# HaoxiangYou/Q_Learning_with_HJB

Measured on AMD Instinct MI355X. Metric: env-steps/sec (batched HJB rollouts), cartpole batch=2^20, higher is better.
Workload: dtype f32; 1 GPU; cartpole balancing + vhjb controller (BASELINE configs[1]); batch_per_gpu=1048576, global_batch=1048576, state_dim=4, control_dim=1, integrator=euler, mlp=4-128-128-64 relu, no bias, parallelism=env-shard x1, no data-path collective

## Files before the change

q_learning_with_hjb_amd/csrc/hjbx_train_coop.hip:

```cpp
#include <hip/hip_runtime.h>
#include <type_traits>

#include "hjbx_internal.hpp"
#include "hjbx_systems.hpp"
#include "hjbx_host.hpp"
#include "hjbx_mlp_core.hpp"
#include "hjbx_adam.hpp"

using namespace hjbx;

static constexpr int kExLd = 33;
static constexpr int kExFloats = 128 * kExLd;
static constexpr int kCoopBlocks = 48;
static constexpr int kCoopSet = 24;
static constexpr int kCoopMaxGrid = 512;

template <int N> struct CoopLds {
    static constexpr int NP = (N + 3) & ~3;
    float W1[N * kLD1];
    float W2[kH1 * kLD2];
    float W3[kH2 * kLD3];
    float E[3][kExFloats];
    __attribute__((aligned(16))) float zs[32 * NP];
    __attribute__((aligned(16))) float gzbs[32 * NP];
    float rs[32];
    float vp[2][32];
    float zeros[32];
    double sums[4][32];
};

template <int AOFF, int BOFF, int ST> __device__ __forceinline__ void coop_issue(float& a, float& b, uint32_t abase, uint32_t bbase) {
    a = lds_read_b32<AOFF * ST>(abase);
    b = lds_read_b32<BOFF * ST>(bbase);
}
struct NoFiller { template <typename I> __device__ __forceinline__ void operator()(I) const {} };
template <int AOFF, int BOFF, int NSTEPS, int DEPTH, int ST, typename Filler>
__device__ __forceinline__ void coop_chain_step(f32x16& acc, float (&ra)[DEPTH + 1], float (&rb)[DEPTH + 1], uint32_t abase, uint32_t bbase, const Filler& filler) {
    if constexpr (ST < NSTEPS) {
        if constexpr (ST + DEPTH < NSTEPS) coop_issue<AOFF, BOFF, ST + DEPTH>(ra[(ST + DEPTH) % (DEPTH + 1)], rb[(ST + DEPTH) % (DEPTH + 1)], abase, bbase);
        __builtin_amdgcn_sched_barrier(0);
        constexpr int ahead = (NSTEPS - 1 - ST < DEPTH ? NSTEPS - 1 - ST : DEPTH) * 2;
        lds_wait<ahead>();
        acc = MFMA(ra[ST % (DEPTH + 1)], rb[ST % (DEPTH + 1)], acc);
        __builtin_amdgcn_sched_barrier(0);
        filler(std::integral_constant<int, ST>{});
        coop_chain_step<AOFF, BOFF, NSTEPS, DEPTH, ST + 1>(acc, ra, rb, abase, bbase, filler);
    }
}
template <int AOFF, int BOFF, int NSTEPS, typename Filler = NoFiller>
__device__ __forceinline__ void coop_chain(f32x16& acc, uint32_t abase, uint32_t bbase, const Filler& filler = Filler()) {
    constexpr int DEPTH = 3;
    static_assert(AOFF * (NSTEPS - 1) < 65536 && BOFF * (NSTEPS - 1) < 65536, "ds_read_b32 offset field is 16 bits");
    float ra[DEPTH + 1], rb[DEPTH + 1];
    coop_issue<AOFF, BOFF, 0>(ra[0], rb[0], abase, bbase);
    if constexpr (NSTEPS > 1) coop_issue<AOFF, BOFF, 1>(ra[1], rb[1], abase, bbase);
    if constexpr (NSTEPS > 2) coop_issue<AOFF, BOFF, 2>(ra[2], rb[2], abase, bbase);
    coop_chain_step<AOFF, BOFF, NSTEPS, DEPTH, 0>(acc, ra, rb, abase, bbase, filler);
}

struct OffW1Fc { static constexpr int at(int st, int) { return 2 * st * kLD1 * 4; } };
struct OffW1Gc { static constexpr int at(int st, int) { return perm(st) * 4; } };

using LP = __attribute__((address_space(3))) float*;
using LPc = const __attribute__((address_space(3))) float*;
__device__ __forceinline__ uint32_t lds_addr(LPc q) { return (uint32_t)(uintptr_t)q; }

__device__ __forceinline__ void zero16(f32x16& a) {
#pragma unroll
    for (int r = 0; r < 16; ++r) a[r] = 0.f;
}

__device__ __forceinline__ void ex_write(LP blk , const f32x16& v) {
#pragma unroll
    for (int r = 0; r < 16; ++r) blk[perm(r) * kExLd] = v[r];
}
__device__ __forceinline__ void ex_add(f32x16& v, LPc blk) {
#pragma unroll
    for (int r = 0; r < 16; ++r) v[r] += blk[perm(r) * kExLd];
}

template <int NB, bool HJB, bool TERM, typename Filler = NoFiller>
__device__ __forceinline__ void coop_outer(f32x16 (&acch)[NB], LPc Ah, LPc Bh, f32x16 (&acct)[NB], LPc At, LPc Bt, LPc rs, int exA, int exBj, int h,
                                           const Filler& filler = Filler()) {
    LPc ah_p = Ah + exA, bh_p = Bh + exBj, at_p = At + exA, bt_p = Bt + exBj, r_p = rs + h;
    struct Ops { float ah, at, rr, bh[NB], bt[NB]; };
    auto load = [&](int s2) __attribute__((always_inline)) {
        Ops o;
        o.ah = o.at = o.rr = 0.f;
        if constexpr (HJB) o.ah = ah_p[2 * s2];
        if constexpr (TERM) { o.at = at_p[2 * s2]; o.rr = r_p[2 * s2]; }
#pragma unroll
        for (int j = 0; j < NB; ++j) {
            o.bh[j] = o.bt[j] = 0.f;
            if constexpr (HJB) o.bh[j] = bh_p[32 * j * kExLd + 2 * s2];
            if constexpr (TERM) o.bt[j] = bt_p[32 * j * kExLd + 2 * s2];
        }
        return o;
    };
    Ops cur = load(0);
#pragma unroll
    for (int s = 0; s < 16; ++s) {
        Ops nxt = cur;
        if (s + 1 < 16) nxt = load(s + 1);
        __builtin_amdgcn_sched_barrier(0);
#pragma unroll
        for (int j = 0; j < NB; ++j) {
            if constexpr (HJB) acch[j] = MFMA(cur.ah, cur.bh[j], acch[j]);
            if constexpr (TERM) acct[j] = MFMA(cur.at, cur.rr * cur.bt[j], acct[j]);
        }
        filler(s);
        __builtin_amdgcn_sched_barrier(0);
        cur = nxt;
    }
}

#ifdef HJBX_COOP_NO_OUTER
#define COOP_OUTER(...)
#else
#define COOP_OUTER(...) __VA_ARGS__
#endif
#ifdef HJBX_COOP_NO_CHAINS
#define COOP_CHAIN(...)
#else
#define COOP_CHAIN(...) __VA_ARGS__
#endif
#ifdef HJBX_COOP_NO_BARRIER
#define COOP_SYNC() __builtin_amdgcn_sched_barrier(0)
#elif defined(HJBX_COOP_STAMPS)
#define COOP_STAMP() do { if (stamp_on) stamp_buf[stamp_idx++] = wall_clock64(); } while (0)
#define COOP_SYNC() do { __syncthreads(); COOP_STAMP(); } while (0)
#else
#define COOP_SYNC() __syncthreads()
#endif
#ifndef COOP_STAMP
#define COOP_STAMP() do { } while (0)
#endif

template <int MODE, int ACT, int PS, typename S>
__global__ __launch_bounds__(256, 1) void k_train_coop(S sys_k, MlpP<S::N> p_k, TaskP<float, S::N, S::M> tk_k, Limits<float, S::M> lim_k,
                                                       const float* __restrict__ W1g, const float* __restrict__ W2g, const float* __restrict__ W3g,
                                                       const float* __restrict__ x, const float* __restrict__ cost, const float* __restrict__ done,
                                                       float eps_term, float* __restrict__ partial, float* __restrict__ partial_w1,
                                                       double* __restrict__ sums_rec, int64_t B, int64_t ntiles) {
    constexpr int N = S::N, M = S::M;
    constexpr int NP = CoopLds<N>::NP;
    static_assert(N % 2 == 0 && N <= HJBX_MAX_N, "state dimension");
    __shared__ __attribute__((aligned(256))) CoopLds<N> L;
    __shared__ __attribute__((aligned(16))) unsigned char sys_raw[sizeof(S)];
    S& sys_s = *reinterpret_cast<S*>(sys_raw);
    __shared__ MlpP<N> p_s;
    __shared__ TaskP<float, N, M> tk_s;
    __shared__ Limits<float, M> lim_s;
    const int tid = threadIdx.x;
#ifdef HJBX_COOP_STAMPS
    const bool stamp_on = PS == 4 && blockIdx.x == 1 && tid == 0;
    unsigned long long* stamp_buf = reinterpret_cast<unsigned long long*>(partial_w1 + (int64_t)blockIdx.x * 2 * (2 * S::N * 128));
    int stamp_idx = 0;
    COOP_STAMP();
#endif
    if (tid == 0) { sys_s = sys_k; p_s = p_k; tk_s = tk_k; lim_s = lim_k; }
#ifndef HJBX_COOP_NO_FILL
    {
        static_assert(kH1 % 4 == 0 && kH2 % 4 == 0 && kH3 % 4 == 0, "");
        const float4* W1v = reinterpret_cast<const float4*>(W1g);
        const float4* W2v = reinterpret_cast<const float4*>(W2g);
        const float4* W3v = reinterpret_cast<const float4*>(W3g);
        auto put4 = [](float* dst, const float4& v) { dst[0] = v.x; dst[1] = v.y; dst[2] = v.z; dst[3] = v.w; };
        constexpr int Q1 = (N * kH1 / 4 + 255) / 256, Q2 = kH1 * kH2 / 4 / 256, Q3 = kH2 * kH3 / 4 / 256;
        static_assert(kH1 * kH2 / 4 % 256 == 0 && kH2 * kH3 / 4 % 256 == 0, "");
        float4 v1[Q1], v2[Q2], v3[Q3];
#pragma unroll
        for (int q = 0; q < Q2; ++q) v2[q] = W2v[tid + 256 * q];
#pragma unroll
        for (int q = 0; q < Q3; ++q) v3[q] = W3v[tid + 256 * q];
#pragma unroll
        for (int q = 0; q < Q1; ++q) v1[q] = tid + 256 * q < N * kH1 / 4 ? W1v[tid + 256 * q] : float4{0.f, 0.f, 0.f, 0.f};
#pragma unroll
        for (int q = 0; q < Q1; ++q) {
            const int idx = tid + 256 * q;
            if (idx < N * kH1 / 4) put4(&L.W1[(idx / (kH1 / 4)) * kLD1 + 4 * (idx % (kH1 / 4))], v1[q]);
        }
#pragma unroll
        for (int q = 0; q < Q2; ++q) { const int idx = tid + 256 * q; put4(&L.W2[(idx / (kH2 / 4)) * kLD2 + 4 * (idx % (kH2 / 4))], v2[q]); }
#pragma unroll
        for (int q = 0; q < Q3; ++q) { const int idx = tid + 256 * q; put4(&L.W3[(idx / (kH3 / 4)) * kLD3 + 4 * (idx % (kH3 / 4))], v3[q]); }
    }
#endif
    if (tid < 32) L.zeros[tid] = 0.f;
    if (tid < 128) L.sums[tid >> 5][tid & 31] = 0.0;
    for (int idx = tid; idx < kExFloats; idx += 256) L.E[2][idx] = 0.f;
    for (int idx = tid; idx < 32 * NP; idx += 256) { L.zs[idx] = 0.f; L.gzbs[idx] = 0.f; }
    __syncthreads();
    COOP_STAMP();
    const S& sys = sys_s;
    const MlpP<N>& p = p_s;
    const TaskP<float, N, M>& tk = tk_s;
    const Limits<float, M>& lim = lim_s;
    const int lane = tid & 63, w = __builtin_amdgcn_readfirstlane(tid >> 6);
    const int i = lane & 31, h = lane >> 5;
    const int ob = w & 1, kh = w >> 1;
    static_assert(PS == 1 || PS == 4, "");
    constexpr int psplit = PS;
    constexpr int NB2 = PS == 4 ? 1 : 4, NB3 = PS == 4 ? 1 : 2;
    const int part = PS == 4 ? (int)(blockIdx.x & 3u) : 0;
    const int col2 = PS == 4 ? 32 * part * kExLd : 0;
    const int col3 = PS == 4 ? 32 * (part & 1) * kExLd : 0;
    const bool do3 = PS == 1 || part < 2;
    const bool own1 = part == 0;
    const float m1 = own1 ? 1.0f : 0.0f;
    auto lds = [](const void* q) { return (uint32_t)(uintptr_t)q; };
    auto lds3 = [](LPc q) { return lds_addr(q); };
    const uint32_t aW1f = lds(&L.W1[h * kLD1 + 32 * w + i]);
    const uint32_t aW1g = i < N ? lds(&L.W1[i * kLD1 + 32 * w + 4 * h]) : lds(&L.zeros[0]);
    const uint32_t aW2f = lds(&L.W2[h * kLD2 + 32 * w + i]);
    const uint32_t aW2b = lds(&L.W2[(32 * w + i) * kLD2 + h]);
    const uint32_t aW3f = lds(&L.W3[(64 * kh + h) * kLD3 + 32 * ob + i]);
    const uint32_t aW3b = lds(&L.W3[(32 * w + i) * kLD3 + h]);
    const LP E0g = (LP)&L.E[0][0], E1g = (LP)&L.E[1][0], E2g = (LP)&L.E[2][0];
    const LP rsg = (LP)&L.rs[0], zsg = (LP)&L.zs[0], gzbsg = (LP)&L.gzbs[0];
    const int exB = h * kExLd + i;
    const int exW = (32 * w + 4 * h) * kExLd + i;
    const int exWy = (32 * ob + 4 * h) * kExLd + i;
    const int exA = (32 * w + i) * kExLd + h;
    const int exO = i * kExLd + h;
    constexpr int AO1 = 2 * kLD2 * 4, AO3 = 2 * kLD3 * 4, BOX = 2 * kExLd * 4;

    f32x16 acc2h[NB2], acc2t[NB2], acc3h[NB3], acc3t[NB3];
#pragma unroll
    for (int j = 0; j < NB2; ++j) { zero16(acc2h[j]); zero16(acc2t[j]); }
#pragma unroll
    for (int j = 0; j < NB3; ++j) { zero16(acc3h[j]); zero16(acc3t[j]); }
    f32x2 w1h[N / 2], w1t[N / 2];
#pragma unroll
    for (int k = 0; k < N / 2; ++k) w1h[k] = w1t[k] = f32x2{0.f, 0.f};
    const int fW1 = tid & 127, sW1 = 16 * (tid >> 7);

    auto fetch = [&](int64_t tile, float (&xv)[N], float& dnv, float& cstv) __attribute__((always_inline)) {
        const int64_t env = tile * 32 + i;
        const bool ok = tile < ntiles && env < B;
        if (ok) load_row<N>(x, env, xv);
        else {
#pragma unroll
            for (int k = 0; k < N; ++k) xv[k] = p.xf[k];
        }
        dnv = ok ? done[env] : 0.f;
        cstv = ok ? cost[env] : 1.f;
    };
    float xs_n[N], dn_n, cst_n;
    const int64_t tile_stride = gridDim.x / (unsigned)psplit;
    fetch(blockIdx.x / (unsigned)psplit, xs_n, dn_n, cst_n);
    for (int64_t tile = blockIdx.x / (unsigned)psplit; tile < ntiles; tile += tile_stride) {
        asm volatile("" ::: "memory");
        LP E0 = E0g, E1 = E1g, E2 = E2g, rsp = rsg, zsp = zsg, gzbsp = gzbsg;
        asm volatile("" : "+v"(E0), "+v"(E1), "+v"(E2), "+v"(rsp), "+v"(zsp), "+v"(gzbsp));
        const bool valid = tile * 32 + i < B;
        float xs[N];
#pragma unroll
        for (int k = 0; k < N; ++k) xs[k] = xs_n[k];
        const float dn = dn_n, cst = cst_n;
        float e[N], z[N], ee = 0.f;
#pragma unroll
        for (int k = 0; k < N; ++k) e[k] = xs[k] - p.xf[k];
        sys.wrap(e);
#pragma unroll
        for (int k = 0; k < N; ++k) {
            ee += e[k] * e[k];
            z[k] = (e[k] - p.mean[k]) * p.istd[k];
        }
        float ring1[3][1];
        f32x16 t[1][1];

        zero_acc(t);
        mfma_chain<OffW1Fc, N / 2, 1, 2, 1>(t, ring1, aW1f, [&](int st, int) { return h ? z[2 * st + 1] : z[2 * st]; });
        constexpr bool SIN = ACT == HJBX_ACT_SIN;
        f32x16 h1r, s1r;
#pragma unroll
        for (int r = 0; r < 16; ++r) {
            if constexpr (SIN) {
                float sn, cs;
                sincos1(t[0][0][r], sn, cs);
                asm volatile("" : "+v"(sn), "+v"(cs));
                h1r[r] = sn;
                s1r[r] = cs;
            } else {
                h1r[r] = act1<ACT>(t[0][0][r]);
            }
        }
        auto dmul1 = [&](int r, float v) __attribute__((always_inline)) { if constexpr (SIN) return v * s1r[r]; else return dact1<ACT>(h1r[r], v); };
        ex_write(E0 + exW, h1r);
        COOP_SYNC();
        f32x16 acc;
        zero16(acc);
        {
            using f32x4 = __attribute__((ext_vector_type(4))) float;
            using LP4 = const __attribute__((address_space(3))) f32x4*;
            LPc a1p = E2 + fW1 * kExLd + sW1;
            const LP4 zz4 = (LP4)(zsp + sW1 * NP);
            auto w1_part2 = [&](auto st_c) __attribute__((always_inline)) {
                constexpr int st = decltype(st_c)::value;
#if !defined(HJBX_COOP_NO_W1) && !defined(HJBX_COOP_NO_FILL2)
                if constexpr (st % 4 == 0) {
                    constexpr int s2 = st / 4;
                    const float a = a1p[s2] * m1;
                    const f32x2 a2v{a, a};
#pragma unroll
                    for (int k4 = 0; k4 < NP / 4; ++k4) {
                        const f32x4 zz = zz4[s2 * (NP / 4) + k4];
#pragma unroll
                        for (int c = 0; c < 2; ++c)
                            if (4 * k4 + 2 * c < N) w1h[2 * k4 + c] = __builtin_elementwise_fma(f32x2{zz[2 * c], zz[2 * c + 1]}, a2v, w1h[2 * k4 + c]);
                    }
#pragma unroll
                    for (int k = 0; k < N / 2; ++k) asm volatile("" : "+v"(w1h[k]));
                }
#endif
            };
#ifdef HJBX_COOP_NO_CHAINS
            (void)w1_part2;
#endif
            COOP_CHAIN(coop_chain<AO1, BOX, 64>(acc, aW2f, lds3(E0 + exB), w1_part2);)
        }
        f32x16 h2r, s2r;
#pragma unroll
        for (int r = 0; r < 16; ++r) {
            if constexpr (SIN) {
                float sn, cs;
                sincos1(acc[r], sn, cs);
                asm volatile("" : "+v"(sn), "+v"(cs));
                h2r[r] = sn;
                s2r[r] = cs;
            } else {
                h2r[r] = act1<ACT>(acc[r]);
            }
        }
        auto dmul2 = [&](int r, float v) __attribute__((always_inline)) { if constexpr (SIN) return v * s2r[r]; else return dact1<ACT>(h2r[r], v); };
        ex_write(E1 + exW, h2r);
        COOP_SYNC();
        zero16(acc);
        COOP_CHAIN(coop_chain<AO3, BOX, 32>(acc, aW3f, lds3(E1 + 64 * kh * kExLd + exB));)
        if (kh == 1) ex_write(E2 + exWy, acc);
        COOP_SYNC();
        f32x16 dyr;
        zero16(dyr);
        if (kh == 0) {
            ex_add(acc, E2 + exWy);
            float vpart = 0.f;
#pragma unroll
            for (int r = 0; r < 16; ++r) {
                vpart += acc[r] * acc[r];
                dyr[r] = acc[r] + acc[r];
            }
            vpart += __shfl_xor(vpart, 32, 64);
            if (h == 0) L.vp[ob][i] = vpart;
            ex_write(E0 + exWy, dyr);
        }
        COOP_SYNC();
        const float V = (L.vp[0][i] + L.vp[1][i]) + p.eps_s * ee;
        float lt, rterm;
        termination_residual_env<float>(eps_term, V, cst, dn, lt, rterm);
        if (!valid) lt = rterm = 0.f;
        if (w == 0 && h == 0) {
            L.rs[i] = rterm;
            if (valid && own1) { L.sums[1][i] += (double)lt; L.sums[2][i] += 1.0 - (double)dn; L.sums[3][i] += (double)dn; }
        }
        zero16(acc);
        COOP_CHAIN(coop_chain<2 * 4, BOX, 32>(acc, aW3b, lds3(E0 + exB));)
        f32x16 d2r;
        f32x16 c2r;
#pragma unroll
        for (int r = 0; r < 16; ++r) {
            d2r[r] = dmul2(r, acc[r]);
            if constexpr (SIN) c2r[r] = -h2r[r] * acc[r];
        }
        ex_write(E1 + exW, d2r);
        COOP_SYNC();
        zero16(acc);
        COOP_CHAIN(coop_chain<2 * 4, BOX, 64>(acc, aW2b, lds3(E1 + exB));)
        f32x16 d1r;
        f32x16 c1r;
#pragma unroll
        for (int r = 0; r < 16; ++r) {
            d1r[r] = dmul1(r, acc[r]);
            if constexpr (SIN) c1r[r] = -h1r[r] * acc[r];
        }
        ex_write(E2 + exW, d1r);
        zero_acc(t);
        mfma_chain<OffW1Gc, 16, 1, 2, 1>(t, ring1, aW1g, [&](int st, int) { return d1r[st]; });
        {
            LP gp = E0 + w * (N * 32) + i;
#pragma unroll
            for (int r = 0; r < 16; ++r) {
                const int k0 = perm(r);
                if (k0 + 4 * h < N && (k0 < N)) gp[(k0 + 4 * h) * 32] = t[0][0][r];
            }
        }
        COOP_SYNC();
        float g[N];
#pragma unroll
        for (int k = 0; k < N; ++k) {
            LPc gp = E0 + k * 32 + i;
            g[k] = ((gp[0] + gp[N * 32]) + (gp[2 * N * 32] + gp[3 * N * 32])) * p.istd[k] + 2.f * p.eps_s * e[k];
        }
        float li, q[N];
#ifdef HJBX_COOP_NO_RESID
        li = g[0];
#pragma unroll
        for (int k = 0; k < N; ++k) q[k] = g[k];
#else
        hjb_residual_env<MODE>(sys, tk, lim, xs, g, dn, true, li, q);
#endif
        if (!valid) {
            li = 0.f;
#pragma unroll
            for (int k = 0; k < N; ++k) q[k] = 0.f;
        }
        float gzb[N];
#pragma unroll
        for (int k = 0; k < N; ++k) gzb[k] = q[k] * p.istd[k];
        if (w == 0 && h == 0) {
            if (valid && own1) L.sums[0][i] += (double)li;
#pragma unroll
            for (int k = 0; k < N; ++k) { L.zs[i * NP + k] = z[k]; L.gzbs[i * NP + k] = gzb[k]; }
        }
        zero_acc(t);
        mfma_chain<OffW1Fc, N / 2, 1, 2, 1>(t, ring1, aW1f, [&](int st, int) { return h ? gzb[2 * st + 1] : gzb[2 * st]; });
        f32x16 dh1b;
#pragma unroll
        for (int r = 0; r < 16; ++r) {
            if constexpr (ACT == HJBX_ACT_TANH) c1r[r] = -2.f * h1r[r] * d1r[r] * t[0][0][r];
            if constexpr (SIN) c1r[r] *= t[0][0][r];
            dh1b[r] = dmul1(r, t[0][0][r]);
        }
        COOP_SYNC();
        ex_write(E0 + exW, dh1b);
        COOP_SYNC();
        using f32x4 = __attribute__((ext_vector_type(4))) float;
        using LP4 = const __attribute__((address_space(3))) f32x4*;
        LPc d1p = E2 + fW1 * kExLd + sW1, rp1 = rsp + sW1;
        const LP4 gz4 = (LP4)(gzbsp + sW1 * NP), zz4 = (LP4)(zsp + sW1 * NP);
        auto w1_part1 = [&](int s2) __attribute__((always_inline)) {
#if !defined(HJBX_COOP_NO_W1) && !defined(HJBX_COOP_NO_FILL1)
            const float d = d1p[s2] * m1;
            const float rd = rp1[s2] * d;
            const f32x2 d2v{d, d}, rd2v{rd, rd};
#pragma unroll
            for (int k4 = 0; k4 < NP / 4; ++k4) {
                const f32x4 gz = gz4[s2 * (NP / 4) + k4];
                const f32x4 zz = zz4[s2 * (NP / 4) + k4];
#pragma unroll
                for (int c = 0; c < 2; ++c)
                    if (4 * k4 + 2 * c < N) {
                        w1h[2 * k4 + c] = __builtin_elementwise_fma(f32x2{gz[2 * c], gz[2 * c + 1]}, d2v, w1h[2 * k4 + c]);
                        w1t[2 * k4 + c] = __builtin_elementwise_fma(f32x2{zz[2 * c], zz[2 * c + 1]}, rd2v, w1t[2 * k4 + c]);
                    }
            }
#pragma unroll
            for (int k = 0; k < N / 2; ++k) asm volatile("" : "+v"(w1h[k]), "+v"(w1t[k]));
#endif
        };
#ifdef HJBX_COOP_NO_OUTER
#pragma unroll
        for (int s2 = 0; s2 < 16; ++s2) w1_part1(s2);
#endif
        COOP_OUTER(coop_outer<NB2, true, false>(acc2h, E0, E1 + col2, acc2t, E0, E1 + col2, rsp, exA, exO, h, w1_part1);)
        zero16(acc);
        COOP_CHAIN(coop_chain<AO1, BOX, 64>(acc, aW2f, lds3(E0 + exB));)
        f32x16 dh2b;
#pragma unroll
        for (int r = 0; r < 16; ++r) {
            if constexpr (ACT == HJBX_ACT_TANH) c2r[r] = -2.f * h2r[r] * d2r[r] * acc[r];
            if constexpr (SIN) c2r[r] *= acc[r];
            dh2b[r] = dmul2(r, acc[r]);
        }
        COOP_SYNC();
        ex_write(E1 + exW, dh2b);
        if (kh == 0) ex_write(E2 + exWy, dyr);
        COOP_SYNC();
        COOP_OUTER(coop_outer<NB3, true, false>(acc3h, E1, E2 + col3, acc3t, E1, E2 + col3, rsp, exA, exO, h);)
        fetch(tile + tile_stride, xs_n, dn_n, cst_n);
        zero16(acc);
        COOP_CHAIN(coop_chain<AO3, BOX, 32>(acc, aW3f, lds3(E1 + 64 * kh * kExLd + exB));)
        if (kh == 1) ex_write(E0 + exWy, acc);
        COOP_SYNC();
        if (kh == 0) {
            ex_add(acc, E0 + exWy);
#pragma unroll
            for (int r = 0; r < 16; ++r) acc[r] += acc[r];
            ex_write(E0 + exWy, acc);
        }
        ex_write(E1 + exW, h2r);
        COOP_SYNC();
        COOP_OUTER(coop_outer<NB3, true, true>(acc3h, E1, E0 + col3, acc3t, E1, E2 + col3, rsp, exA, exO, h);)
        zero16(acc);
        COOP_CHAIN(coop_chain<2 * 4, BOX, 32>(acc, aW3b, lds3(E0 + exB));)
        f32x16 a2b;
#pragma unroll
        for (int r = 0; r < 16; ++r) {
            a2b[r] = dmul2(r, acc[r]);
            if constexpr (ACT != HJBX_ACT_RELU) a2b[r] += c2r[r];
        }
        COOP_SYNC();
        ex_write(E2 + exW, a2b);
        ex_write(E1 + exW, h1r);
        ex_write(E0 + exW, d2r);
        COOP_SYNC();
        COOP_OUTER(coop_outer<NB2, true, true>(acc2h, E1, E2 + col2, acc2t, E1, E0 + col2, rsp, exA, exO, h);)
        zero16(acc);
        COOP_CHAIN(coop_chain<2 * 4, BOX, 64>(acc, aW2b, lds3(E2 + exB));)
        f32x16 a1b;
#pragma unroll
        for (int r = 0; r < 16; ++r) {
            a1b[r] = dmul1(r, acc[r]);
            if constexpr (ACT != HJBX_ACT_RELU) a1b[r] += c1r[r];
        }
        COOP_SYNC();
        ex_write(E2 + exW, a1b);
    }
    COOP_SYNC();
    {
        using f32x4 = __attribute__((ext_vector_type(4))) float;
        using LP4 = const __attribute__((address_space(3))) f32x4*;
        LPc a1p = E2g + fW1 * kExLd + sW1;
        const LP4 zz4 = (LP4)(zsg + sW1 * NP);
#ifndef HJBX_COOP_NO_W1
#pragma unroll 4
        for (int s2 = 0; s2 < 16; ++s2) {
            const float a = a1p[s2] * m1;
            const f32x2 a2v{a, a};
#pragma unroll
            for (int k4 = 0; k4 < NP / 4; ++k4) {
                const f32x4 zz = zz4[s2 * (NP / 4) + k4];
#pragma unroll
                for (int c = 0; c < 2; ++c)
                    if (4 * k4 + 2 * c < N) w1h[2 * k4 + c] = __builtin_elementwise_fma(f32x2{zz[2 * c], zz[2 * c + 1]}, a2v, w1h[2 * k4 + c]);
            }
        }
#endif
    }
    COOP_STAMP();
    float* out = partial + (int64_t)blockIdx.x * kCoopBlocks * 1024;
    auto put = [&](int blk, const f32x16& a) {
#pragma unroll
        for (int r = 0; r < 16; ++r) out[blk * 1024 + r * 64 + lane] = a[r];
    };
    if constexpr (PS == 4) {
        put(w * 4 + part, acc2h[0]);
        put(kCoopSet + w * 4 + part, acc2t[0]);
        if (do3) {
            put(16 + w * 2 + (part & 1), acc3h[0]);
            put(kCoopSet + 16 + w * 2 + (part & 1), acc3t[0]);
        }
    } else {
#pragma unroll
        for (int j = 0; j < NB2; ++j) { put(w * 4 + j, acc2h[j]); put(kCoopSet + w * 4 + j, acc2t[j]); }
#pragma unroll
        for (int j = 0; j < NB3; ++j) { put(16 + w * 2 + j, acc3h[j]); put(kCoopSet + 16 + w * 2 + j, acc3t[j]); }
    }
    if (own1) {
        float* o1 = partial_w1 + ((int64_t)blockIdx.x * 2 + (tid >> 7)) * (2 * N * 128);
#pragma unroll
        for (int k = 0; k < N; ++k) { o1[k * 128 + fW1] = w1h[k >> 1][k & 1]; o1[(N + k) * 128 + fW1] = w1t[k >> 1][k & 1]; }
    }
    if (w == 0 && own1) {
        double acc_h = h == 0 ? L.sums[0][i] : 0.0, acc_t = h == 0 ? L.sums[1][i] : 0.0;
        double acc_ni = h == 0 ? L.sums[2][i] : 0.0, acc_nd = h == 0 ? L.sums[3][i] : 0.0;
#pragma unroll
        for (int off = 32; off > 0; off >>= 1) {
            acc_h += __shfl_down(acc_h, off, 64); acc_t += __shfl_down(acc_t, off, 64);
            acc_ni += __shfl_down(acc_ni, off, 64); acc_nd += __shfl_down(acc_nd, off, 64);
        }
        if (lane == 0) {
            double* rec = sums_rec + 4 * (int64_t)blockIdx.x;
            rec[0] = acc_h; rec[1] = acc_t; rec[2] = acc_ni; rec[3] = acc_nd;
        }
    }
    COOP_STAMP();
#ifdef HJBX_COOP_STAMPS
    if (stamp_on) stamp_buf[63] = (unsigned long long)stamp_idx;
#endif
}

__device__ __forceinline__ float coop_sum8(const float* __restrict__ base, int64_t stride, int count) {
    float s8[8] = {0.f, 0.f, 0.f, 0.f, 0.f, 0.f, 0.f, 0.f};
    int gI = 0;
    for (; gI + 8 <= count; gI += 8) {
#pragma unroll
        for (int k = 0; k < 8; ++k) s8[k] += base[(int64_t)(gI + k) * stride];
    }
    for (int k = 0; gI < count; ++gI, ++k) s8[k] += base[(int64_t)gI * stride];
    return ((s8[0] + s8[1]) + (s8[2] + s8[3])) + ((s8[4] + s8[5]) + (s8[6] + s8[7]));
}
__device__ __forceinline__ void coop_sum8x2(const float* __restrict__ a, const float* __restrict__ b, int64_t stride, int count, float& sa, float& sb) {
    float p[8] = {0.f, 0.f, 0.f, 0.f, 0.f, 0.f, 0.f, 0.f}, q[8] = {0.f, 0.f, 0.f, 0.f, 0.f, 0.f, 0.f, 0.f};
    int gI = 0;
    for (; gI + 8 <= count; gI += 8) {
        float va[8], vb[8];
#pragma unroll
        for (int k = 0; k < 8; ++k) { va[k] = a[(int64_t)(gI + k) * stride]; vb[k] = b[(int64_t)(gI + k) * stride]; }
#pragma unroll
        for (int k = 0; k < 8; ++k) { p[k] += va[k]; q[k] += vb[k]; }
    }
    for (int k = 0; gI < count; ++gI, ++k) { p[k] += a[(int64_t)gI * stride]; q[k] += b[(int64_t)gI * stride]; }
    sa = ((p[0] + p[1]) + (p[2] + p[3])) + ((p[4] + p[5]) + (p[6] + p[7]));
    sb = ((q[0] + q[1]) + (q[2] + q[3])) + ((q[4] + q[5]) + (q[6] + q[7]));
}

template <int N> __device__ __forceinline__ float coop_sum_w1(const float* __restrict__ base , int nparts, int psplit) {
    if (psplit != 4) return coop_sum8(base, 2 * N * 128, 2 * nparts);
    float s0, s1;
    coop_sum8x2(base, base + 2 * N * 128, (int64_t)8 * (2 * N * 128), nparts / 4, s0, s1);
    return s0 + s1;
}

struct CoopOwners { int first, step, count; };
__device__ __forceinline__ CoopOwners coop_owners(int b , int nparts, int psplit) {
    if (psplit != 4) return CoopOwners{0, 1, nparts};
    const int jb = b < 0 ? 0 : (b < 16 ? (b & 3) : ((b - 16) & 1));
    return CoopOwners{jb, 4, nparts / 4};
}

template <int N>
__global__ __launch_bounds__(256) void k_train_coop_reduce(const float* __restrict__ partial, const float* __restrict__ partial_w1, int nparts, int psplit,
                                                          const double* __restrict__ sums_rec, float* __restrict__ flat) {
    constexpr int P = N * kH1 + kH1 * kH2 + kH2 * kH3;
    const int t = blockIdx.x * 256 + threadIdx.x;
    if (t < kCoopBlocks * 1024) {
        const CoopOwners ow = coop_owners((t >> 10) % kCoopSet, nparts, psplit);
        const float s = coop_sum8(partial + (int64_t)ow.first * kCoopBlocks * 1024 + t, (int64_t)ow.step * kCoopBlocks * 1024, ow.count);
        const int blk = t >> 10, reg = (t >> 6) & 15, lane = t & 63;
        const int row = (reg & 3) + 8 * (reg >> 2) + 4 * (lane >> 5), col = lane & 31;
        const int set = blk / kCoopSet, b = blk % kCoopSet;
        float* o = flat + set * P;
        if (b < 16) o[N * kH1 + (32 * (b >> 2) + row) * kH2 + 32 * (b & 3) + col] = s;
        else o[N * kH1 + kH1 * kH2 + (32 * ((b - 16) >> 1) + row) * kH3 + 32 * ((b - 16) & 1) + col] = s;
    } else if (t < kCoopBlocks * 1024 + 2 * N * 128) {
        const int u = t - kCoopBlocks * 1024;
        const int set = u / (N * 128), kf = u % (N * 128);
        flat[set * P + kf] = coop_sum_w1<N>(partial_w1 + u, nparts, psplit);
    } else if (t < kCoopBlocks * 1024 + 2 * N * 128 + 4) {
        const int k = t - (kCoopBlocks * 1024 + 2 * N * 128);
        const CoopOwners ow = coop_owners(-1, nparts, psplit);
        double s = 0;
        for (int g = 0; g < ow.count; ++g) s += sums_rec[4 * (ow.first + g * ow.step) + k];
        flat[2 * P + k] = (float)s;
    }
}

template <int N>
__global__ __launch_bounds__(256) void k_train_coop_update(const float* __restrict__ partial, const float* __restrict__ partial_w1, int nparts, int psplit,
                                                          const double* __restrict__ sums_rec, AdamArgs a, MixArgs mx, GatherArgs next) {
    __shared__ float sc[2];
    __shared__ double tot[4];
    __shared__ double rec[4 * kCoopMaxGrid];
    const float tstep = adam_coef_begin(a, sc);
    for (int idx = threadIdx.x; idx < 4 * nparts; idx += 256) rec[idx] = sums_rec[idx];
    const int t = blockIdx.x * 256 + threadIdx.x;
    float sh = 0.f, st = 0.f;
    int which = -1;
    int64_t j = 0;
    if (t < kCoopSet * 1024) {
        const int b = t >> 10, reg16 = (t >> 6) & 15, lane = t & 63;
        const CoopOwners ow = coop_owners(b, nparts, psplit);
        const float* src = partial + (int64_t)ow.first * kCoopBlocks * 1024 + t;
        coop_sum8x2(src, src + kCoopSet * 1024, (int64_t)ow.step * kCoopBlocks * 1024, ow.count, sh, st);
        const int row = (reg16 & 3) + 8 * (reg16 >> 2) + 4 * (lane >> 5), col = lane & 31;
        if (b < 16) { which = 1; j = (int64_t)(32 * (b >> 2) + row) * kH2 + 32 * (b & 3) + col; }
        else { which = 2; j = (int64_t)(32 * ((b - 16) >> 1) + row) * kH3 + 32 * ((b - 16) & 1) + col; }
    } else if (t < kCoopSet * 1024 + N * 128) {
        const int kf = t - kCoopSet * 1024;
        sh = coop_sum_w1<N>(partial_w1 + kf, nparts, psplit);
        st = coop_sum_w1<N>(partial_w1 + N * 128 + kf, nparts, psplit);
        which = 0; j = kf;
    }
    __syncthreads();
    if (threadIdx.x < 4) {
        const CoopOwners ow = coop_owners(-1, nparts, psplit);
        double s = 0;
        for (int g = 0; g < ow.count; ++g) s += rec[4 * (ow.first + g * ow.step) + threadIdx.x];
        tot[threadIdx.x] = (double)(float)s;
    }
    __syncthreads();
    const AdamCoef c = adam_coef_end(a, tstep, sc);
    const float reg = mx.reg_dev ? mx.reg_dev[0] : mx.reg_host;
    const float ih = 1.0f / ((float)tot[2] + mx.eps), it = 1.0f / ((float)tot[3] + mx.eps);
    const float wt = reg * it;
    if (which >= 0) adam_element(a, c, which, j, sh * ih + st * wt);
    const int64_t k_next = next.enabled && mx.step_counter ? (int64_t)mx.step_counter[0] + 1 : 0;
    if (next.enabled) gather_elements(next, k_next, (int64_t)blockIdx.x * 256 + threadIdx.x, (int64_t)gridDim.x * 256);
    if (adam_finish(a, c, mx, (float)tot[0] * ih, (float)tot[1] * it, reg) && next.enabled) gather_reg(next, k_next);
}

struct CoopWs { size_t partial, partial_w1, sums, total; int grid, psplit; };
static CoopWs coop_ws(int64_t B, int n) {
    CoopWs w{};
    int n_cu = hjbx_device_cus();
    if (n_cu <= 0) n_cu = 256;
    const int64_t ntiles = (B + 31) / 32;
    w.psplit = 4 * ntiles <= n_cu ? 4 : 1;
    w.grid = (int)(ntiles * w.psplit < n_cu ? ntiles * w.psplit : n_cu);
    auto up = [](size_t v) { return (v + 255) & ~(size_t)255; };
    w.partial = up((size_t)w.grid * kCoopBlocks * 1024 * sizeof(float));
    w.partial_w1 = up((size_t)w.grid * 2 * 2 * n * 128 * sizeof(float));
    w.sums = up((size_t)w.grid * 4 * sizeof(double));
    w.total = w.partial + w.partial_w1 + w.sums;
    return w;
}

size_t hjbx_train_coop_workspace_bytes(int64_t B, int n) { return B > 0 ? coop_ws(B, n).total : 0; }

template <typename S>
static int launch_coop(const hjbx_system* sysh, S sys, const hjbx_task* task, const hjbx_mlp* mlp, int mode, const float* x, const float* cost,
                       const float* done, float* flat, void* workspace, int64_t B, void* st, const FuseArgs* fuse) {
    constexpr int N = S::N, M = S::M;
    if constexpr (N % 2 != 0 || N > HJBX_MAX_N) {
        return HJBX_EUNSUPPORTED;
    } else {
        if (hjbx_device_cus() <= 0) return hjbx_set_error(HJBX_ENODEVICE, "hjbx_value_loss_grad_f32: no HIP device");
        MlpP<N> p;
        for (int k = 0; k < N; ++k) { p.mean[k] = (float)mlp->mean[k]; p.istd[k] = (float)(1.0 / mlp->std[k]); p.xf[k] = (float)mlp->xf[k]; }
        p.eps_s = (float)mlp->eps_scalar;
        const auto tk = make_task<float, N, M>(task);
        const auto lim = make_limits<float, M>(sysh);
        const CoopWs w = coop_ws(B, N);
        float* partial = (float*)workspace;
        float* partial_w1 = (float*)((char*)workspace + w.partial);
        double* sums = (double*)((char*)workspace + w.partial + w.partial_w1);
        const int64_t ntiles = (B + 31) / 32;
        const float *W1 = (const float*)mlp->W1, *W2 = (const float*)mlp->W2, *W3 = (const float*)mlp->W3;
        hipStream_t s = (hipStream_t)st;
        auto go = [&](auto mode_c, auto act_c) {
            if (w.psplit == 4)
                hipLaunchKernelGGL((k_train_coop<decltype(mode_c)::value, decltype(act_c)::value, 4, S>), dim3(w.grid), dim3(256), 0, s, sys, p, tk, lim, W1, W2, W3,
                                   x, cost, done, (float)task->eps, partial, partial_w1, sums, B, ntiles);
            else
                hipLaunchKernelGGL((k_train_coop<decltype(mode_c)::value, decltype(act_c)::value, 1, S>), dim3(w.grid), dim3(256), 0, s, sys, p, tk, lim, W1, W2, W3,
                                   x, cost, done, (float)task->eps, partial, partial_w1, sums, B, ntiles);
        };
        auto with_act = [&](auto mode_c) {
            if (mlp->activation == HJBX_ACT_TANH) go(mode_c, std::integral_constant<int, HJBX_ACT_TANH>{});
            else if (mlp->activation == HJBX_ACT_SIN) {
                if constexpr (N <= 4) go(mode_c, std::integral_constant<int, HJBX_ACT_SIN>{});
            }
            else go(mode_c, std::integral_constant<int, HJBX_ACT_RELU>{});
        };
        if (mode == HJBX_RESIDUAL_NORMALISED) with_act(std::integral_constant<int, 0>{});
        else with_act(std::integral_constant<int, 1>{});
        if (fuse) {
            if (fuse->a.end0 != N * kH1 || fuse->a.end1 - fuse->a.end0 != kH1 * kH2 || fuse->a.P - fuse->a.end1 != kH2 * kH3)
                return hjbx_set_error(HJBX_EINVAL, "hjbx_value_loss_adam_f32: the Adam state's tensors must be W1 (%d x 128), W2 (128 x 128), W3 (128 x 64)", N);
            if (w.grid > kCoopMaxGrid) return hjbx_set_error(HJBX_EUNSUPPORTED, "hjbx_value_loss_adam_f32: %d workgroups (more than %d CUs?)", w.grid, kCoopMaxGrid);
            const int nthreads = kCoopSet * 1024 + N * 128;
            hipLaunchKernelGGL((k_train_coop_update<N>), dim3((nthreads + 255) / 256), dim3(256), 0, s, partial, partial_w1, w.grid, w.psplit, sums, fuse->a, fuse->mx, fuse->next);
        } else {
            const int nthreads = kCoopBlocks * 1024 + 2 * N * 128 + 4;
            hipLaunchKernelGGL((k_train_coop_reduce<N>), dim3((nthreads + 255) / 256), dim3(256), 0, s, partial, partial_w1, w.grid, w.psplit, sums, flat);
        }
        hipError_t e = hipGetLastError();
        if (e != hipSuccess) return hjbx_set_error(HJBX_EHIP, "hjbx_value_loss_grad_f32: %s", hipGetErrorString(e));
        return HJBX_OK;
    }
}

int hjbx_train_coop(const hjbx_system* sys, const hjbx_task* task, const hjbx_mlp* mlp, int mode, const float* x, const float* cost, const float* done,
                    float* flat, void* workspace, int64_t B, void* stream, const FuseArgs* fuse) {
    if (mlp->activation == HJBX_ACT_SIN && sys->n > 4)
        return hjbx_set_error(HJBX_EUNSUPPORTED, "hjbx_value_loss_grad_f32: the sin network's fused parameter gradient exists for n <= 4 (n = %d)", sys->n);
    int rc = HJBX_EUNSUPPORTED;
#ifdef HJBX_TRAIN_DEV
    bool ok = false;
    if (sys->kind == HJBX_SYS_CARTPOLE) {
        Cartpole<float> cp{(float)sys->p[0], (float)sys->p[1], (float)sys->p[2], (float)sys->p[3]};
        rc = launch_coop<Cartpole<float>>(sys, cp, task, mlp, mode, x, cost, done, flat, workspace, B, stream, fuse);
        ok = true;
    } else if (sys->kind == HJBX_SYS_NEARHOVER) {
        NearHover<float> q{(float)sys->p[0], (float)sys->p[1], (float)sys->p[2], (float)sys->p[3]};
        rc = launch_coop<NearHover<float>>(sys, q, task, mlp, mode, x, cost, done, flat, workspace, B, stream, fuse);
        ok = true;
    }
#else
    const bool ok = with_system<float>(sys, [&](auto S) { rc = launch_coop<decltype(S)>(sys, S, task, mlp, mode, x, cost, done, flat, workspace, B, stream, fuse); });
#endif
    if (!ok || rc == HJBX_EUNSUPPORTED)
        return hjbx_set_error(HJBX_EUNSUPPORTED, "hjbx_value_loss_grad_f32: no kernel for system kind %d with n=%d m=%d", sys->kind, sys->n, sys->m);
    return rc;
}
```

Measured before the change: 1.428 billion env-steps/s.

## Hoist termination-term outer products into the residual phase to hide MFMAs

The termination-gradient outer products (acct) no longer ride alongside the HJB outer products. They are now computed separately right after the partial-gradient sync, using pre-scaled r*dy and r*d2 images written to spare LDS regions. A sched_group_barrier pattern interleaves these MFMAs with the scalar VALU work of the HJB residual, and the E-buffer writes are reshuffled so one sync-guarded exchange goes away. The aim is to hide MFMA latency under the residual math and to lighten the later outer-product loops. In exchange the LDS buffers are reused more aggressively and register pressure goes up during the residual phase.

New measurement: 1.428 billion env-steps/s. No clear change (-0.0%).

```diff
diff --git a/q_learning_with_hjb_amd/csrc/hjbx_train_coop.hip b/q_learning_with_hjb_amd/csrc/hjbx_train_coop.hip
--- a/q_learning_with_hjb_amd/csrc/hjbx_train_coop.hip
+++ b/q_learning_with_hjb_amd/csrc/hjbx_train_coop.hip
@@ -79,22 +79,15 @@
     for (int r = 0; r < 16; ++r) v[r] += blk[perm(r) * kExLd];
 }
 
-template <int NB, bool HJB, bool TERM, typename Filler = NoFiller>
-__device__ __forceinline__ void coop_outer(f32x16 (&acch)[NB], LPc Ah, LPc Bh, f32x16 (&acct)[NB], LPc At, LPc Bt, LPc rs, int exA, int exBj, int h,
-                                           const Filler& filler = Filler()) {
-    LPc ah_p = Ah + exA, bh_p = Bh + exBj, at_p = At + exA, bt_p = Bt + exBj, r_p = rs + h;
-    struct Ops { float ah, at, rr, bh[NB], bt[NB]; };
+template <int NB, typename Filler = NoFiller>
+__device__ __forceinline__ void coop_outer(f32x16 (&acc)[NB], LPc A, LPc B, int exA, int exBj, const Filler& filler = Filler()) {
+    LPc a_p = A + exA, b_p = B + exBj;
+    struct Ops { float a, b[NB]; };
     auto load = [&](int s2) __attribute__((always_inline)) {
         Ops o;
-        o.ah = o.at = o.rr = 0.f;
-        if constexpr (HJB) o.ah = ah_p[2 * s2];
-        if constexpr (TERM) { o.at = at_p[2 * s2]; o.rr = r_p[2 * s2]; }
-#pragma unroll
-        for (int j = 0; j < NB; ++j) {
-            o.bh[j] = o.bt[j] = 0.f;
-            if constexpr (HJB) o.bh[j] = bh_p[32 * j * kExLd + 2 * s2];
-            if constexpr (TERM) o.bt[j] = bt_p[32 * j * kExLd + 2 * s2];
-        }
+        o.a = a_p[2 * s2];
+#pragma unroll
+        for (int j = 0; j < NB; ++j) o.b[j] = b_p[32 * j * kExLd + 2 * s2];
         return o;
     };
     Ops cur = load(0);
@@ -104,15 +97,29 @@
         if (s + 1 < 16) nxt = load(s + 1);
         __builtin_amdgcn_sched_barrier(0);
 #pragma unroll
-        for (int j = 0; j < NB; ++j) {
-            if constexpr (HJB) acch[j] = MFMA(cur.ah, cur.bh[j], acch[j]);
-            if constexpr (TERM) acct[j] = MFMA(cur.at, cur.rr * cur.bt[j], acct[j]);
-        }
+        for (int j = 0; j < NB; ++j) acc[j] = MFMA(cur.a, cur.b[j], acc[j]);
         filler(s);
         __builtin_amdgcn_sched_barrier(0);
         cur = nxt;
     }
 }
+
+template <int NB> __device__ __forceinline__ void coop_outer_term(f32x16 (&acc)[NB], LPc a_p, LPc b_p) {
+#pragma unroll
+    for (int s = 0; s < 16; ++s) {
+        const float a = a_p[2 * s];
+#pragma unroll
+        for (int j = 0; j < NB; ++j) acc[j] = MFMA(a, b_p[32 * j * kExLd + 2 * s], acc[j]);
+    }
+}
+template <int NM> __device__ __forceinline__ void coop_shadow_schedule() {
+#pragma unroll
+    for (int m = 0; m < NM; ++m) {
+        __builtin_amdgcn_sched_group_barrier(0x008, 1, 0);
+        __builtin_amdgcn_sched_group_barrier(0x002, 10, 0);
+    }
+}
+static constexpr int kExRdy = 40;
 
 #ifdef HJBX_COOP_NO_OUTER
 #define COOP_OUTER(...)
@@ -363,6 +370,12 @@
             L.rs[i] = rterm;
             if (valid && own1) { L.sums[1][i] += (double)lt; L.sums[2][i] += 1.0 - (double)dn; L.sums[3][i] += (double)dn; }
         }
+        if (kh == 0) {
+            f32x16 rdy;
+#pragma unroll
+            for (int r = 0; r < 16; ++r) rdy[r] = rterm * dyr[r];
+            ex_write(E2 + kExRdy * kExLd + exWy, rdy);
+        }
         zero16(acc);
         COOP_CHAIN(coop_chain<2 * 4, BOX, 32>(acc, aW3b, lds3(E0 + exB));)
         f32x16 d2r;
@@ -383,11 +396,17 @@
             d1r[r] = dmul1(r, acc[r]);
             if constexpr (SIN) c1r[r] = -h1r[r] * acc[r];
         }
-        ex_write(E2 + exW, d1r);
         zero_acc(t);
         mfma_chain<OffW1Gc, 16, 1, 2, 1>(t, ring1, aW1g, [&](int st, int) { return d1r[st]; });
         {
-            LP gp = E0 + w * (N * 32) + i;
+            f32x16 rd2;
+#pragma unroll
+            for (int r = 0; r < 16; ++r) rd2[r] = rterm * d2r[r];
+            ex_write(E0 + exW, rd2);
+        }
+        {
+            static_assert(4 * N * 32 <= kExRdy * kExLd && kExRdy + 64 <= 128, "partial g and the r dy image share E2");
+            LP gp = E2 + w * (N * 32) + i;
 #pragma unroll
             for (int r = 0; r < 16; ++r) {
                 const int k0 = perm(r);
@@ -395,12 +414,15 @@
             }
         }
         COOP_SYNC();
+        __builtin_amdgcn_sched_barrier(0);
         float g[N];
 #pragma unroll
         for (int k = 0; k < N; ++k) {
-            LPc gp = E0 + k * 32 + i;
+            LPc gp = E2 + k * 32 + i;
             g[k] = ((gp[0] + gp[N * 32]) + (gp[2 * N * 32] + gp[3 * N * 32])) * p.istd[k] + 2.f * p.eps_s * e[k];
         }
+        LPc tA = E1 + exA, tB2 = E0 + col2 + exO, tB3 = E2 + kExRdy * kExLd + col3 + exO;
+        asm volatile("" : "+v"(tA), "+v"(tB2), "+v"(tB3));
         float li, q[N];
 #ifdef HJBX_COOP_NO_RESID
         li = g[0];
@@ -409,14 +431,28 @@
 #else
         hjb_residual_env<MODE>(sys, tk, lim, xs, g, dn, true, li, q);
 #endif
-        if (!valid) {
-            li = 0.f;
-#pragma unroll
-            for (int k = 0; k < N; ++k) q[k] = 0.f;
-        }
+#pragma unroll
+        for (int k = 0; k < N; ++k) asm volatile("" : "+v"(q[k]));
+        li = valid ? li : 0.f;
         float gzb[N];
 #pragma unroll
-        for (int k = 0; k < N; ++k) gzb[k] = q[k] * p.istd[k];
+        for (int k = 0; k < N; ++k) gzb[k] = (valid ? q[k] : 0.f) * p.istd[k];
+        ex_write(E1 + exW, h1r);
+#ifdef X_PINNED
+        COOP_OUTER(coop_outer<NB2>(acc2t, E1, E0 + col2, exA, exO);)
+#else
+        COOP_OUTER(coop_outer_term<NB2>(acc2t, tA, tB2);)
+#endif
+        ex_write(E1 + exW, h2r);
+#ifdef X_PINNED
+        COOP_OUTER(coop_outer<NB3>(acc3t, E1, E2 + kExRdy * kExLd + col3, exA, exO);)
+#else
+        COOP_OUTER(coop_outer_term<NB3>(acc3t, tA, tB3);)
+#endif
+#if !defined(X_PINNED) && !defined(X_NOSG)
+        COOP_OUTER(coop_shadow_schedule<16 * (NB2 + NB3)>();)
+#endif
+        __builtin_amdgcn_sched_barrier(0);
         if (w == 0 && h == 0) {
             if (valid && own1) L.sums[0][i] += (double)li;
 #pragma unroll
@@ -433,6 +469,8 @@
         }
         COOP_SYNC();
         ex_write(E0 + exW, dh1b);
+        ex_write(E1 + exW, d2r);
+        ex_write(E2 + exW, d1r);
         COOP_SYNC();
         using f32x4 = __attribute__((ext_vector_type(4))) float;
         using LP4 = const __attribute__((address_space(3))) f32x4*;
@@ -462,7 +500,7 @@
 #pragma unroll
         for (int s2 = 0; s2 < 16; ++s2) w1_part1(s2);
 #endif
-        COOP_OUTER(coop_outer<NB2, true, false>(acc2h, E0, E1 + col2, acc2t, E0, E1 + col2, rsp, exA, exO, h, w1_part1);)
+        COOP_OUTER(coop_outer<NB2>(acc2h, E0, E1 + col2, exA, exO, w1_part1);)
         zero16(acc);
         COOP_CHAIN(coop_chain<AO1, BOX, 64>(acc, aW2f, lds3(E0 + exB));)
         f32x16 dh2b;
@@ -476,7 +514,7 @@
         ex_write(E1 + exW, dh2b);
         if (kh == 0) ex_write(E2 + exWy, dyr);
         COOP_SYNC();
-        COOP_OUTER(coop_outer<NB3, true, false>(acc3h, E1, E2 + col3, acc3t, E1, E2 + col3, rsp, exA, exO, h);)
+        COOP_OUTER(coop_outer<NB3>(acc3h, E1, E2 + col3, exA, exO);)
         fetch(tile + tile_stride, xs_n, dn_n, cst_n);
         zero16(acc);
         COOP_CHAIN(coop_chain<AO3, BOX, 32>(acc, aW3f, lds3(E1 + 64 * kh * kExLd + exB));)
@@ -490,7 +528,7 @@
         }
         ex_write(E1 + exW, h2r);
         COOP_SYNC();
-        COOP_OUTER(coop_outer<NB3, true, true>(acc3h, E1, E0 + col3, acc3t, E1, E2 + col3, rsp, exA, exO, h);)
+        COOP_OUTER(coop_outer<NB3>(acc3h, E1, E0 + col3, exA, exO);)
         zero16(acc);
         COOP_CHAIN(coop_chain<2 * 4, BOX, 32>(acc, aW3b, lds3(E0 + exB));)
         f32x16 a2b;
@@ -502,9 +540,8 @@
         COOP_SYNC();
         ex_write(E2 + exW, a2b);
         ex_write(E1 + exW, h1r);
-        ex_write(E0 + exW, d2r);
-        COOP_SYNC();
-        COOP_OUTER(coop_outer<NB2, true, true>(acc2h, E1, E2 + col2, acc2t, E1, E0 + col2, rsp, exA, exO, h);)
+        COOP_SYNC();
+        COOP_OUTER(coop_outer<NB2>(acc2h, E1, E2 + col2, exA, exO);)
         zero16(acc);
         COOP_CHAIN(coop_chain<2 * 4, BOX, 64>(acc, aW2b, lds3(E2 + exB));)
         f32x16 a1b;
```
